# BVE-Reborn/rend3

Measured on AMD Instinct MI355X. Metric: shaded Mpixels/s @4K (whole frame: cull+compact all cameras, 4 shadow views, PBR opaque, tonemap), higher is better.
Workload: dtype f32; 1 GPU; BASELINE.json configs[2] stand-in: bistro_like (seed 0xB157, every object owns its geometry), 3840x2160, full PBR opaque + 4 directional shadow views (2048^2), camera dolly, 130 materials with base colour + normal + AO/roughness/metallic maps (RGBA8, mips, trilinear); objects=3000, triangles=2823212, cameras=5, parallelism=single GPU

## Files before the change

rend3_amd/csrc/kernels_shade.h:

```cpp
#pragma once
#include <type_traits>

#include "device_math.h"
#include "texture.h"

#define R3N_TEX_OCC 5
#define R3N_MS_OCC 4

struct TriRecord;
struct ViewLights;
struct ShadeArgs {
    const unsigned long long *vis;
    uint32_t width, height, row_begin, row_end;
    const r3n_frame_uniforms496 *fu;
    const r3n_camera_header240 *hdr;
    const r3n_object128 *objects;
    const uint32_t *mesh;
    const r3n_baked128 *baked;
    const r3n_material208 *materials;
    uint32_t n_materials;
    const uint32_t *tri_base;
    const uint32_t *slot_table;
    uint32_t slot_table_size;
    const uint8_t *dir_buf;
    const uint8_t *point_buf;
    const float *atlas;
    uint32_t atlas_w, atlas_h;
    float clear[4];
    ushort4 *hdr_out;
    uchar4 *ldr_out;
    const unsigned char *srgb_lut;
    bool out_bgr;
    TextureArgs tex;
    ushort4 *samples_out;
    TriRecord *tri_rec;
    unsigned char *seen;
    uint32_t total_tris;
    uint32_t *edge_list, *edge_count;
    uint32_t edge_capacity;
    const ViewLights *view_lights;
    const uint32_t *material_feat;
    uint32_t variants;
    uint32_t resolve_lds;
};
#define R3N_EDGEQ 32u

#define R3N_FEAT_TEX_ALBEDO   0x001u
#define R3N_FEAT_TEX_NORMAL   0x002u
#define R3N_FEAT_TEX_AOMR     0x004u
#define R3N_FEAT_TEX_AOMR_X   0x008u
#define R3N_FEAT_TEX_MISC     0x010u
#define R3N_FEAT_VCOLOR       0x020u
#define R3N_FEAT_UNLIT        0x040u
#define R3N_FEAT_NEAREST      0x080u
#define R3N_FEAT_AOMR_SPLIT   0x100u
#define R3N_FEAT_CLEARCOAT    0x200u
#define R3N_FEAT_NORMAL_FLAGS 0x400u
#define R3N_FEAT_ALBEDO_OFF   0x800u
#define R3N_FEAT_TEX_GENERAL  0x1000u
#define R3N_FEAT_ALL          0x1FFFu
#define R3N_BATCH_OCC 4
#define R3N_CLS_PLAIN  0u
#define R3N_CLS_ALBEDO (R3N_FEAT_TEX_ALBEDO)
#define R3N_CLS_PBR3   (R3N_FEAT_TEX_ALBEDO | R3N_FEAT_TEX_NORMAL | R3N_FEAT_TEX_AOMR)
#define R3N_CLS_ALL    R3N_FEAT_ALL
#define R3N_VARIANTS 4u
static inline uint32_t r3n_material_features(const r3n_material208 &m) {
    const uint32_t f = m.flags;
    uint32_t k = 0;
    if (m.textures[0]) k |= R3N_FEAT_TEX_ALBEDO;
    if (m.textures[1]) k |= R3N_FEAT_TEX_NORMAL;
    if (m.textures[2]) k |= R3N_FEAT_TEX_AOMR;
    if (m.textures[3] || m.textures[9]) k |= R3N_FEAT_TEX_AOMR_X;
    if (m.textures[4] || m.textures[5] || m.textures[6] || m.textures[7]) k |= R3N_FEAT_TEX_MISC;
    if (f & R3N_FLAGS_ALBEDO_BLEND) k |= R3N_FEAT_VCOLOR;
    if (f & R3N_FLAGS_UNLIT) k |= R3N_FEAT_UNLIT;
    if (f & R3N_FLAGS_NEAREST) k |= R3N_FEAT_NEAREST;
    if ((m.textures[2] || m.textures[3] || m.textures[9]) && !(f & R3N_FLAGS_AOMR_COMBINED)) k |= R3N_FEAT_AOMR_SPLIT;
    if (!(m.clear_coat == 0.0f)) k |= R3N_FEAT_CLEARCOAT;
    if (f & (R3N_FLAGS_BICOMPONENT_NORMAL | R3N_FLAGS_SWIZZLED_NORMAL | R3N_FLAGS_YDOWN_NORMAL)) k |= R3N_FEAT_NORMAL_FLAGS;
    if (!(f & R3N_FLAGS_ALBEDO_ACTIVE)) k |= R3N_FEAT_ALBEDO_OFF;
    return k;
}
#if defined(__HIPCC__)
__host__ __device__
#endif
static inline uint32_t r3n_variant_of(uint32_t feat) {
    if (feat & ~R3N_CLS_PBR3) return 3u;
    if (feat & ~R3N_CLS_ALBEDO) return 2u;
    return feat ? 1u : 0u;
}

struct TriRecord {
    float e[3][3];
    float vp[3][4];
    float vn[3][3];
    float vt[3][3];
    float vc[3][4];
    float uv[3][2];
    uint32_t object, material;
    uint32_t feat;
    uint32_t _pad[4];
};
static_assert(sizeof(TriRecord) == 256, "triangle record is 64 dwords");

struct BlendApplyArgs {
    const unsigned long long *keys;
    const uint32_t *vals;
    const uint32_t *head;
    uint32_t first_sample, n_samples;
    uint32_t capacity;
    ushort4 *samples;
};

#define R3N_SRGB_LUT_SIZE 0x3C00u

struct LdsDirLight {
    float m[16];
    float l[3];
    float color[3];
    float inv_res[2], offset[2], size[2];
    float sane;
    float _pad[3];
};
static_assert(sizeof(LdsDirLight) == 128, "two s_load_dwordx16");
struct LdsPointLight {
    float vpos[3];
    float color[3];
    float radius;
    float _pad;
};
static_assert(sizeof(LdsPointLight) == 32, "one s_load_dwordx8");
struct ViewLights {
    uint32_t n_dir, n_point, _pad[2];
    LdsDirLight dir[R3N_MAX_DIR_LIGHTS];
    LdsPointLight point[R3N_MAX_POINT_LIGHTS];
};

#ifndef R3N_SHADE_DECL_ONLY

struct PcfTap {
    int ix, iy;
    float fx, fy;
};
R3N_DEV PcfTap pcf_tap(uint32_t aw, uint32_t ah, float u, float v, int ox, int oy) {
    const float tx = (u * (float)aw - 0.5f) + (float)ox;
    const float ty = (v * (float)ah - 0.5f) + (float)oy;
    const float fx0 = floorf(tx), fy0 = floorf(ty);
    PcfTap t;
    t.fx = tx - fx0; t.fy = ty - fy0;
    t.ix = (fx0 == fx0 && fabsf(fx0) < 1e9f) ? (int)fx0 : 0;
    t.iy = (fy0 == fy0 && fabsf(fy0) < 1e9f) ? (int)fy0 : 0;
    if (!(t.fx == t.fx)) t.fx = 0.0f;
    if (!(t.fy == t.fy)) t.fy = 0.0f;
    return t;
}
R3N_DEV uint32_t wrap_texel(int v, uint32_t n) {
    if ((uint32_t)v < n) return (uint32_t)v;
    const long long w = (long long)n;
    return (uint32_t)((((long long)v % w) + w) % w);
}
R3N_DEV float pcf_texel_cmp(const float *__restrict__ atlas, uint32_t aw, uint32_t ah, int x, int y, float ref) {
    return ref >= atlas[(size_t)wrap_texel(y, ah) * aw + wrap_texel(x, aw)] ? 1.0f : 0.0f;
}

template <class M>
R3N_DEV float shadow_pcf5_general(const float *__restrict__ atlas, uint32_t aw, uint32_t ah, float u, float v, float ref) {
    float r = 0.0f;
#pragma unroll 1
    for (int k = 0; k < 5; ++k) {
        const int ox = k == 3 ? 1 : (k == 4 ? -1 : 0), oy = k == 1 ? 1 : (k == 2 ? -1 : 0);
        const PcfTap t = pcf_tap(aw, ah, u, v, ox, oy);
        float c[4];
#pragma unroll 1
        for (int j = 0; j < 4; ++j) c[j] = pcf_texel_cmp(atlas, aw, ah, t.ix + (j & 1), t.iy + (j >> 1), ref);
        const f2 tb = M::mad((f2){c[1], c[3]}, splat2(t.fx), (f2){c[0], c[2]} * splat2(1.0f - t.fx));
        r = r + M::mad(tb.y, t.fy, tb.x * (1.0f - t.fy));
    }
    return r * 0.2f;
}

template <class M>
R3N_DEV float shadow_pcf5(const float *__restrict__ atlas, uint32_t aw, uint32_t ah, float u, float v, float ref) {
    const float tx0 = u * (float)aw - 0.5f, ty0 = v * (float)ah - 0.5f;
    const float txp = tx0 + 1.0f, txm = tx0 + -1.0f, typ = ty0 + 1.0f, tym = ty0 + -1.0f;
    const float f0x = floorf(tx0), fpx = floorf(txp), fmx = floorf(txm);
    const float f0y = floorf(ty0), fpy = floorf(typ), fmy = floorf(tym);
// ... 69 lines not shown
    const float x = 1.0f - loh, x2 = x * x, x5 = (x2 * x2) * x;
    const float ggxl = nov * M::sqrt(M::mad(M::mad(-nol, a2, nol), nol, a2));
    const float ggxv = nol * (pre ? pre->sqrt_v : M::sqrt(M::mad(M::mad(-nov, a2, nov), nov, a2)));
    const float vis = M::half_over(ggxl + ggxv);
    const float k = nol * occlusion;
    const float dv = d * vis;
    {
        const f2 f0 = {px.f0[0], px.f0[1]};
        const f2 fres = M::mad(splat2(f90) - f0, splat2(x5), f0);
        const f2 color = M::mad(splat2(dv), fres, (f2){px.diffuse[0], px.diffuse[1]} * splat2(1.0f / R3N_PI));
        const f2 o = (color * (f2){intensity[0], intensity[1]}) * splat2(k);
        out[0] = o.x; out[1] = o.y;
    }
    {
        const float fres = M::mad(f90 - px.f0[2], x5, px.f0[2]);
        const float color = M::mad(dv, fres, px.diffuse[2] * (1.0f / R3N_PI));
        out[2] = (color * intensity[2]) * k;
    }
}

R3N_DEV float srgb_to_linear(float e) { return e > 0.04045f ? powf((e + 0.055f) / 1.055f, 2.4f) : e / 12.92f; }

R3N_DEV float srgb_oetf(float x) {
    if (!(x > 0.0f)) return 0.0f;
    if (x >= 1.0f) return 1.0f;
    if (x <= 0.0031308f) return x * 12.92f;
    return 1.055f * powf(x, 1.0f / 2.4f) - 0.055f;
}
static __global__ __launch_bounds__(256) void k_build_srgb_lut(unsigned char *__restrict__ lut) {
    const uint32_t h = blockIdx.x * 256u + threadIdx.x;
    if (h >= R3N_SRGB_LUT_SIZE) return;
    const float x = (float)__builtin_bit_cast(_Float16, (unsigned short)h);
    lut[h] = (unsigned char)(srgb_oetf(x) * 255.0f + 0.5f);
}
R3N_DEV unsigned char srgb8_of_half(const unsigned char *__restrict__ lut, unsigned short h) {
    if (h & 0x8000u) return 0;
    if (h > 0x7C00u) return 0;
    if (h >= R3N_SRGB_LUT_SIZE) return 255;
    return lut[h];
}
R3N_DEV uchar4 tonemap_half4(const unsigned char *__restrict__ lut, ushort4 h, bool bgr = false) {
    const float al = (float)__builtin_bit_cast(_Float16, h.w);
    const float a = (!(al > 0.0f)) ? 0.0f : (al >= 1.0f ? 1.0f : al);
    const unsigned char r = srgb8_of_half(lut, h.x), g = srgb8_of_half(lut, h.y), b = srgb8_of_half(lut, h.z);
    return make_uchar4(bgr ? b : r, g, bgr ? r : b, (unsigned char)(a * 255.0f + 0.5f));
}
R3N_DEV float srgb_scene_to_display(float x) {
    const float e = x > 0.0031308f ? 1.055f * powf(x, 0.4166f) - 0.055f : x * 12.92f;
    if (!(e > 0.0f)) return 0.0f;
    return e >= 1.0f ? 1.0f : e;
}

R3N_DEV ushort4 pack_half4(const float v[4]) {
    ushort4 o;
    o.x = __builtin_bit_cast(unsigned short, (_Float16)v[0]);
    o.y = __builtin_bit_cast(unsigned short, (_Float16)v[1]);
    o.z = __builtin_bit_cast(unsigned short, (_Float16)v[2]);
    o.w = __builtin_bit_cast(unsigned short, (_Float16)v[3]);
    return o;
}


template <bool TEX>
R3N_DEV void vertex_stage(const ShadeArgs &a, uint32_t id, TriRecord &r) {
    const uint32_t slot = id - 1u;
    const uint32_t bucket = slot >> R3N_SLOT_TABLE_SHIFT;
    uint32_t lo = a.slot_table[bucket];
    uint32_t hi = bucket + 1u < a.slot_table_size ? a.slot_table[bucket + 1u] + 1u : a.hdr->object_count;
    while (hi - lo > 1u) {
        const uint32_t mid = lo + (hi - lo) / 2u;
        if (a.tri_base[mid] <= slot) lo = mid; else hi = mid;
    }
    const uint32_t obj = lo, tri = slot - a.tri_base[obj];
    const r3n_object128 &ob = a.objects[obj];
    const uint4 of0 = *reinterpret_cast<const uint4 *>(reinterpret_cast<const char *>(&ob) + 80);
    const uint4 of1 = *reinterpret_cast<const uint4 *>(reinterpret_cast<const char *>(&ob) + 96);
    const uint32_t of5 = ob.vertex_attribute_start_offsets[5];
    const uint32_t mat_index = of0.z < a.n_materials ? of0.z : 0u;
    const r3n_material208 &mat = a.materials[mat_index];
    const float *mv = a.baked[obj].model_view;
    r.object = obj;
    r.material = mat_index;
    r.feat = a.material_feat != nullptr ? a.material_feat[mat_index] : R3N_FEAT_ALL;

    uint32_t idx[3];
    float p[3][4];
    const float inv_s2[3] = {1.0f / dot3(mv, mv), 1.0f / dot3(mv + 4, mv + 4), 1.0f / dot3(mv + 8, mv + 8)};
    const uint32_t first = of0.x + tri * 3u;
    const uint32_t pos_off = of0.w;
    const uint32_t nrm_off = of1.x;
    const uint32_t tan_off = of1.y;
    const uint32_t uv0_off = of1.z;
    const uint32_t col_off = of5;
    bool any_tex = false, normal_map = false;
    if (TEX) {
        const uint4 t0 = *reinterpret_cast<const uint4 *>(&mat.textures[0]), t1 = *reinterpret_cast<const uint4 *>(&mat.textures[4]);
        const uint2 t2 = *reinterpret_cast<const uint2 *>(&mat.textures[8]);
        any_tex = (((t0.x | t0.y) | (t0.z | t0.w)) | ((t1.x | t1.y) | (t1.z | t1.w)) | (t2.x | t2.y)) != 0u;
        normal_map = t0.y != 0u;
    }
    fetch_indices3(a.mesh, first, idx);
#pragma unroll
    for (int k = 0; k < 3; ++k) {
        float v[3];
        fetch_vec3(a.mesh, pos_off, idx[k], v);
        mul_point(a.baked[obj].model_view_proj, v, p[k]);
        mul_point(mv, v, r.vp[k]);
        float nm[3] = {0.0f, 0.0f, 0.0f};
        if (nrm_off != R3N_INVALID) fetch_vec3(a.mesh, nrm_off, idx[k], nm);
        const float sn[3] = {inv_s2[0] * nm[0], inv_s2[1] * nm[1], inv_s2[2] * nm[2]};
        mat3_mul_vec3(mv, mv + 4, mv + 8, sn, r.vn[k]);
        normalize3(r.vn[k]);
        if (TEX && normal_map) {
            float tg[3] = {0.0f, 0.0f, 0.0f};
            if (tan_off != R3N_INVALID) fetch_vec3(a.mesh, tan_off, idx[k], tg);
            const float st[3] = {inv_s2[0] * tg[0], inv_s2[1] * tg[1], inv_s2[2] * tg[2]};
            mat3_mul_vec3(mv, mv + 4, mv + 8, st, r.vt[k]);
            normalize3(r.vt[k]);
        } else {
            r.vt[k][0] = r.vt[k][1] = r.vt[k][2] = 0.0f;
        }
        if (col_off != R3N_INVALID) {
            const uint32_t cw = a.mesh[col_off / 4u + idx[k]];
#pragma unroll
            for (int c = 0; c < 4; ++c) r.vc[k][c] = (float)((cw >> (8 * c)) & 0xFFu) / 255.0f;
        } else {
#pragma unroll
            for (int c = 0; c < 4; ++c) r.vc[k][c] = 1.0f;
        }
        if (TEX && any_tex) fetch_uv0(a.mesh, uv0_off, idx[k], r.uv[k]);
        else r.uv[k][0] = r.uv[k][1] = 0.0f;
    }
    TriSetup ts;
    setup_triangle(p, (float)a.width / 2.0f, (float)a.height / 2.0f,
                   (a.hdr->flags & R3N_PCU_POSITIVE_AREA_VISIBLE) != 0u, ts);
#pragma unroll
    for (int i = 0; i < 3; ++i)
#pragma unroll
        for (int c = 0; c < 3; ++c) r.e[i][c] = ts.e[i][c];
}

template <class M> R3N_DEV f2 interp2(const float lam[3], f2 a0, f2 a1, f2 a2) {
    return M::mad(splat2(lam[2]), a2, M::mad(splat2(lam[1]), a1, splat2(lam[0]) * a0));
}
template <class M> R3N_DEV float interp1(const float lam[3], float a0, float a1, float a2) {
    return M::mad(lam[2], a2, M::mad(lam[1], a1, lam[0] * a0));
}
template <class M> R3N_DEV void interp_vec3(const float lam[3], const float a[3][3], float o[3]) {
    const f2 xy = interp2<M>(lam, (f2){a[0][0], a[0][1]}, (f2){a[1][0], a[1][1]}, (f2){a[2][0], a[2][1]});
    o[0] = xy.x; o[1] = xy.y;
    o[2] = interp1<M>(lam, a[0][2], a[1][2], a[2][2]);
}
template <class M> R3N_DEV void interp_vec4(const float lam[3], const float a[3][4], float o[4]) {
    const f2 xy = interp2<M>(lam, (f2){a[0][0], a[0][1]}, (f2){a[1][0], a[1][1]}, (f2){a[2][0], a[2][1]});
    const f2 zw = interp2<M>(lam, (f2){a[0][2], a[0][3]}, (f2){a[1][2], a[1][3]}, (f2){a[2][2], a[2][3]});
    o[0] = xy.x; o[1] = xy.y; o[2] = zw.x; o[3] = zw.y;
}

template <class T, bool SL> R3N_DEV T load_light(const T *p) {
#if defined(__HIP_DEVICE_COMPILE__)
    if (SL) {
        static_assert(sizeof(T) % 4 == 0, "whole dwords");
        const unsigned long long v = (unsigned long long)p;
        const uint32_t lo = (uint32_t)__builtin_amdgcn_readfirstlane((uint32_t)v), hi = (uint32_t)__builtin_amdgcn_readfirstlane((uint32_t)(v >> 32));
        typedef __attribute__((address_space(4))) const uint32_t *sp_t;
        const sp_t sp = (sp_t)(((unsigned long long)hi << 32) | (unsigned long long)lo);
        union { T t; uint32_t w[sizeof(T) / 4]; } u;
#pragma unroll
        for (unsigned k = 0; k < sizeof(T) / 4; ++k) u.w[k] = sp[k];
        return u.t;
    }
#endif
    return *p;
}
template <bool TEX, class M = MathExact, uint32_t CLS = R3N_CLS_ALL, bool SL = false>
R3N_DEV void fragment_stage(const ShadeArgs &a, const LdsDirLight *s_dir, const LdsPointLight *s_point, uint32_t n_dir,
                            uint32_t n_point, const TriRecord &r, uint32_t x, uint32_t y, float out[4]) {
    const r3n_material208 &mat = a.materials[r.material];
    constexpr bool kVColor = (CLS & R3N_FEAT_VCOLOR) != 0u, kUnlit = (CLS & R3N_FEAT_UNLIT) != 0u, kNearest = (CLS & R3N_FEAT_NEAREST) != 0u;
    constexpr bool kSplit = (CLS & R3N_FEAT_AOMR_SPLIT) != 0u, kNormalFlags = (CLS & R3N_FEAT_NORMAL_FLAGS) != 0u;
    constexpr bool kAlbedoOff = (CLS & R3N_FEAT_ALBEDO_OFF) != 0u, kMisc = (CLS & R3N_FEAT_TEX_MISC) != 0u;
    constexpr bool kClearCoat = (CLS & (R3N_FEAT_CLEARCOAT | R3N_FEAT_TEX_MISC)) != 0u;
    constexpr bool kAnyTex = TEX && (CLS & (R3N_FEAT_TEX_ALBEDO | R3N_FEAT_TEX_NORMAL | R3N_FEAT_TEX_AOMR | R3N_FEAT_TEX_AOMR_X | R3N_FEAT_TEX_MISC)) != 0u;
    constexpr uint32_t kSlotFeat[10] = {R3N_FEAT_TEX_ALBEDO, R3N_FEAT_TEX_NORMAL, R3N_FEAT_TEX_AOMR, R3N_FEAT_TEX_AOMR_X, R3N_FEAT_TEX_MISC,
                                        R3N_FEAT_TEX_MISC, R3N_FEAT_TEX_MISC, R3N_FEAT_TEX_MISC, R3N_FEAT_TEX_MISC ,
                                        R3N_FEAT_TEX_AOMR_X};
    TriSetup ts;
#pragma unroll
    for (int i = 0; i < 3; ++i)
#pragma unroll
        for (int c = 0; c < 3; ++c) ts.e[i][c] = r.e[i][c];
    ts.z[0] = ts.z[1] = ts.z[2] = 0.0f; ts.det = 1.0f; ts.valid = true;
    float E[3];
    (void)edge_eval(ts, (float)x + 0.5f, (float)y + 0.5f, E);
    const float rs = exact_math::rcp((E[0] + E[1]) + E[2]);
    const float lam[3] = {E[0] * rs, E[1] * rs, E[2] * rs};
    float vpos[4], nrm[3], col[4] = {1.0f, 1.0f, 1.0f, 1.0f};
    interp_vec4<MathExact>(lam, r.vp, vpos);
    interp_vec3<M>(lam, r.vn, nrm);
    if (kVColor && (mat.flags & R3N_FLAGS_ALBEDO_ACTIVE) && (mat.flags & R3N_FLAGS_ALBEDO_BLEND))
        interp_vec4<M>(lam, r.vc, col);

    PixelData px;
    const uint32_t mflags = mat.flags;
    bool any_tex = false;
    if (kAnyTex) {
#pragma unroll
        for (int k = 0; k < 10; ++k)
            if (CLS & kSlotFeat[k]) any_tex = any_tex || mat.textures[k] != 0u;
    }
    float coords[2] = {0.0f, 0.0f}, ddx[2] = {0.0f, 0.0f}, ddy[2] = {0.0f, 0.0f};
    const bool nearest = kNearest && (mflags & R3N_FLAGS_NEAREST) != 0u;
    if (kAnyTex && any_tex) {
        const f2 sr = interp2<M>(lam, (f2){r.uv[0][0], r.uv[0][1]}, (f2){r.uv[1][0], r.uv[1][1]}, (f2){r.uv[2][0], r.uv[2][1]});
        const float self_raw[2] = {sr.x, sr.y};
        frag_coords<M>(ts, r.uv, mat.uv_transform0, (int)x, (int)y, coords, ddx, ddy, self_raw);
    }
    constexpr bool kShortOnly = (CLS & (R3N_FEAT_TEX_GENERAL | R3N_FEAT_NEAREST)) == 0u;
    constexpr bool kShare = kShortOnly && (CLS & (R3N_FEAT_TEX_NORMAL | R3N_FEAT_TEX_AOMR)) != 0u;
    TexShare tshare;
    tshare.width = 0u; tshare.height = 0u; tshare.mips = 0u; tshare.level = 0u; tshare.frac = 0.0f;
    auto tex4 = [&](int slot, float dst[4]) { tex_sample_grad<M, true, kShortOnly, kShare>(a.tex, mat.textures[slot], nearest, coords[0], coords[1], ddx, ddy, dst, &tshare); };
    auto tex3 = [&](int slot, float dst[4]) { tex_sample_grad<M, false, kShortOnly, kShare>(a.tex, mat.textures[slot], nearest, coords[0], coords[1], ddx, ddy, dst, &tshare); };
    auto has = [&](int slot) { return TEX && (CLS & kSlotFeat[slot]) != 0u && mat.textures[slot] != 0u; };
    constexpr bool kBatch = TEX && kShortOnly && CLS == R3N_CLS_PBR3;
    float tb3[3][4];
    bool batched = false;
    if (kBatch && any_tex) {
        const uint32_t ids[3] = {mat.textures[0], mat.textures[1], mat.textures[2]};
        batched = tex_sample3_batched<M>(a.tex, ids, coords[0], coords[1], ddx, ddy, tb3);
    }
    auto tex_slot012 = [&](int slot, float dst[4], bool need_a) {
        if (kBatch && batched) {
#pragma unroll
            for (int c = 0; c < 4; ++c) dst[c] = tb3[slot][c];
        } else if (need_a) tex4(slot, dst);
        else tex3(slot, dst);
    };
    if (!kAlbedoOff || (mflags & R3N_FLAGS_ALBEDO_ACTIVE)) {
#pragma unroll
        for (int c = 0; c < 4; ++c) px.albedo[c] = 1.0f;
        if (has(0)) tex_slot012(0, px.albedo, true);
        if (kVColor && (mflags & R3N_FLAGS_ALBEDO_BLEND)) {
            if (mflags & R3N_FLAGS_ALBEDO_VERTEX_SRGB) {
#pragma unroll
                for (int c = 0; c < 3; ++c) px.albedo[c] *= srgb_to_linear(col[c]);
                px.albedo[3] *= col[3];
            } else {
#pragma unroll
                for (int c = 0; c < 4; ++c) px.albedo[c] *= col[c];
            }
        }
    } else {
        px.albedo[0] = px.albedo[1] = px.albedo[2] = 0.0f;
        px.albedo[3] = 1.0f;
    }
    {
        const f2 rg = (f2){px.albedo[0], px.albedo[1]} * (f2){mat.albedo[0], mat.albedo[1]};
        const f2 ba = (f2){px.albedo[2], px.albedo[3]} * (f2){mat.albedo[2], mat.albedo[3]};
        px.albedo[0] = rg.x; px.albedo[1] = rg.y; px.albedo[2] = ba.x; px.albedo[3] = ba.y;
    }

    if (kUnlit && (mflags & R3N_FLAGS_UNLIT)) {
#pragma unroll
        for (int c = 0; c < 4; ++c) out[c] = px.albedo[c];
    } else {
        if (has(1)) {
            float t[4], n[3];
            tex_slot012(1, t, true);
            if (kNormalFlags && (mflags & R3N_FLAGS_BICOMPONENT_NORMAL)) {
                float b0 = (mflags & R3N_FLAGS_SWIZZLED_NORMAL) ? t[3] : t[0], b1 = t[1];
                b0 = M::mad(b0, 2.0f, -1.0f);
                b1 = M::mad(b1, 2.0f, -1.0f);
                n[0] = b0; n[1] = b1;
                n[2] = M::sqrt((1.0f - b0 * b0) - b1 * b1);
            } else {
#pragma unroll
                for (int c = 0; c < 3; ++c) n[c] = M::mad(t[c], 2.0f, -1.0f);
                normalize3m<M>(n);
            }
            if (kNormalFlags && (mflags & R3N_FLAGS_YDOWN_NORMAL)) n[1] = -n[1];
            float tng[3];
            interp_vec3<M>(lam, r.vt, tng);
            float nn[3] = {nrm[0], nrm[1], nrm[2]};
            normalize3m<M>(nn);
            normalize3m<M>(tng);
            const float bt[3] = {nn[1] * tng[2] - tng[1] * nn[2], nn[2] * tng[0] - tng[2] * nn[0], nn[0] * tng[1] - tng[0] * nn[1]};
            mat3_mul_vec3m<M>(tng, bt, nn, n, px.normal);
        } else {
#pragma unroll
            for (int c = 0; c < 3; ++c) px.normal[c] = nrm[c];
        }
        normalize3m<M>(px.normal);
        float ao = mat.ambient_occlusion, pr = mat.roughness, metallic = mat.metallic;
        if (!kSplit || (mflags & R3N_FLAGS_AOMR_COMBINED)) {
            if (has(2)) {
                float t[4];
                tex_slot012(2, t, false);
                ao = mat.ambient_occlusion * t[0];
                pr = mat.roughness * t[1];
                metallic = mat.metallic * t[2];
            }
        } else if (mflags & R3N_FLAGS_AOMR_BW_SPLIT) {
            float t[4];
            if (has(2)) { tex3(2, t); pr = mat.roughness * t[0]; }
            if (has(3)) { tex3(3, t); metallic = mat.metallic * t[0]; }
            if (has(9)) { tex3(9, t); ao = mat.ambient_occlusion * t[0]; }
        } else {
            float t[4];
            if (has(2)) {
                tex3(2, t);
                const bool sw = (mflags & R3N_FLAGS_AOMR_SWIZZLED_SPLIT) != 0u;
                pr = mat.roughness * (sw ? t[1] : t[0]);
                metallic = mat.metallic * (sw ? t[2] : t[1]);
// ... 46 lines not shown
#pragma unroll
        for (int c = 0; c < 3; ++c) vv[c] = -vv[c];
        float color[3] = {px.emissive[0], px.emissive[1], px.emissive[2]};
        const float mag = (((fabsf(px.normal[0]) + fabsf(px.normal[1])) + (fabsf(px.normal[2]) + fabsf(vv[0]))) +
                           ((fabsf(vv[1]) + fabsf(vv[2])) + (fabsf(px.f0[0]) + fabsf(px.f0[1])))) +
                          (((fabsf(px.f0[2]) + fabsf(px.diffuse[0])) + (fabsf(px.diffuse[1]) + fabsf(px.diffuse[2]))) + fabsf(px.ao));
        const bool skip_ok = px.roughness >= 1e-9f && px.roughness <= 1e9f && mag < 1e30f;
        const BrdfPixel pre_v = brdf_pixel<M>(px, vv);
        const BrdfPixel *pre = &pre_v;
        for (uint32_t i = 0; i < n_dir; ++i) {
            const LdsDirLight L = load_light<LdsDirLight, SL>(s_dir + i);
            const float nl_raw = dot3m<M>(px.normal, L.l);
            if (px.roughness > 0.0f && nl_raw == nl_raw && sat(nl_raw) == 0.0f) {
#pragma unroll
                for (int c = 0; c < 3; ++c) color[c] += 0.0f;
                continue;
            }
            float sn[4];
            mul_vec4m<MathExact>(L.m, vpos[0], vpos[1], vpos[2], vpos[3], sn);
            const float fl[2] = {sn[0] * 0.5f + 0.5f, sn[1] * 0.5f + 0.5f};
            const float local[2] = {fl[0], 1.0f - fl[1]};
            float tl[2] = {L.offset[0], L.offset[1]};
            float tr[2] = {tl[0] + L.size[0], tl[1] + L.size[1]};
            const float coords[2] = {tl[0] * (1.0f - local[0]) + tr[0] * local[0],
                                     tl[1] * (1.0f - local[1]) + tr[1] * local[1]};
            const float border[2] = {L.inv_res[0] * 1.5f, L.inv_res[1] * 1.5f};
            tl[0] += border[0]; tl[1] += border[1];
            tr[0] -= border[0]; tr[1] -= border[1];
            float shadow = 1.0f;
            if ((fl[0] >= tl[0] || fl[1] >= tl[1]) && (fl[0] <= tr[0] || fl[1] <= tr[1]) && sn[2] >= 0.0f && sn[2] <= 1.0f)
                shadow = shadow_pcf5<M>(a.atlas, a.atlas_w, a.atlas_h, coords[0], coords[1], sn[2]);
            if (skip_ok && L.sane != 0.0f && shadow * px.ao == 0.0f) {
#pragma unroll
                for (int c = 0; c < 3; ++c) color[c] += 0.0f;
                continue;
            }
            float res[3];
            surface_shading<M>(L.l, L.color, px, vv, shadow * px.ao, res, pre);
#pragma unroll
            for (int c = 0; c < 3; ++c) color[c] += res[c];
        }
        for (uint32_t i = 0; i < n_point; ++i) {
            const LdsPointLight P = load_light<LdsPointLight, SL>(s_point + i);
            const float delta[3] = {P.vpos[0] - vpos[0], P.vpos[1] - vpos[1], P.vpos[2] - vpos[2]};
            const float d = M::sqrt(dot3m<M>(delta, delta));
            const float s = sat(M::div(d, P.radius));
            const float s2 = s * s, is2 = 1.0f - s2;
            const float att = M::div(is2 * is2, 1.0f + s2);
            const float inten[3] = {P.color[0] * att, P.color[1] * att, P.color[2] * att};
            const float l[3] = {M::div(delta[0], d), M::div(delta[1], d), M::div(delta[2], d)};
            float res[3];
            surface_shading<M>(l, inten, px, vv, px.ao, res, pre);
#pragma unroll
            for (int c = 0; c < 3; ++c) color[c] += (res[c] > 0.0f ? res[c] : 0.0f);
        }
#pragma unroll
        for (int c = 0; c < 3; ++c) out[c] = fmaxf(a.fu->ambient[c] * px.albedo[c], color[c]);
        out[3] = fmaxf(a.fu->ambient[3] * px.albedo[3], px.albedo[3]);
    }
}

template <bool TEX, class M = MathExact>
R3N_DEV void shade_fragment(const ShadeArgs &a, const LdsDirLight *s_dir, const LdsPointLight *s_point, uint32_t n_dir,
                            uint32_t n_point, uint32_t id, uint32_t x, uint32_t y, float out[4]) {
    TriRecord r;
    vertex_stage<TEX>(a, id, r);
    fragment_stage<TEX, M>(a, s_dir, s_point, n_dir, n_point, r, x, y, out);
}

static __global__ __launch_bounds__(256) void k_mark_visible(const unsigned long long *__restrict__ vis, unsigned char *__restrict__ seen,
                                                      size_t first_pixel, size_t n_pixels) {
    const size_t i = (size_t)blockIdx.x * 256u + threadIdx.x;
    const uint32_t id = i < n_pixels ? (uint32_t)(vis[first_pixel + i] & 0xFFFFFFFFull) : 0u;
    const uint32_t left = (uint32_t)__builtin_amdgcn_update_dpp((int)~id, (int)id, 0x111, 0xF, 0xF, false);
    if (id != 0u && id != left) seen[id - 1u] = 1;
}
template <bool TEX>
__global__ __launch_bounds__(256) void k_vertex_stage(ShadeArgs a) {
    const uint32_t slot = blockIdx.x * 256u + threadIdx.x;
    if (slot >= a.total_tris || !a.seen[slot]) return;
    a.seen[slot] = 0;
    TriRecord r;
    vertex_stage<TEX>(a, slot + 1u, r);
    r._pad[0] = r._pad[1] = r._pad[2] = r._pad[3] = 0u;
    a.tri_rec[slot] = r;
}

R3N_DEV void stage_lights(const ShadeArgs &a, LdsDirLight *s_dir, LdsPointLight *s_point, uint32_t &n_dir, uint32_t &n_point) {
    n_dir = min(*reinterpret_cast<const uint32_t *>(a.dir_buf), (uint32_t)R3N_MAX_DIR_LIGHTS);
    n_point = min(*reinterpret_cast<const uint32_t *>(a.point_buf), (uint32_t)R3N_MAX_POINT_LIGHTS);

    const r3n_dir_light128 *dirs = reinterpret_cast<const r3n_dir_light128 *>(a.dir_buf + 16);
    const r3n_point_light32 *points = reinterpret_cast<const r3n_point_light32 *>(a.point_buf + 16);
    for (uint32_t i = threadIdx.x; i < n_dir * 4u; i += 256u) {
        const uint32_t li = i >> 2, c = i & 3u;
        const float *col = a.fu->inv_view + 4 * c;
        float o[4];
        mul_vec4(dirs[li].view_proj, col[0], col[1], col[2], col[3], o);
#pragma unroll
        for (int r = 0; r < 4; ++r) s_dir[li].m[4 * c + r] = o[r];
        if (c == 0) {
            const float nd[3] = {-dirs[li].direction[0], -dirs[li].direction[1], -dirs[li].direction[2]};
            float l[3];
            mat3_mul_vec3(a.fu->view, a.fu->view + 4, a.fu->view + 8, nd, l);
            normalize3(l);
#pragma unroll
            for (int r = 0; r < 3; ++r) { s_dir[li].l[r] = l[r]; s_dir[li].color[r] = dirs[li].color[r]; }
            s_dir[li].sane = (fabsf(dirs[li].color[0]) <= 1e6f && fabsf(dirs[li].color[1]) <= 1e6f && fabsf(dirs[li].color[2]) <= 1e6f &&
                              fabsf(l[0]) <= 2.0f && fabsf(l[1]) <= 2.0f && fabsf(l[2]) <= 2.0f) ? 1.0f : 0.0f;
#pragma unroll
            for (int r = 0; r < 2; ++r) {
                s_dir[li].inv_res[r] = dirs[li].inv_resolution[r];
                s_dir[li].offset[r] = dirs[li].atlas_offset[r];
                s_dir[li].size[r] = dirs[li].atlas_size[r];
            }
        }
    }
    for (uint32_t i = threadIdx.x; i < n_point; i += 256u) {
        float o[4];
        mul_vec4(a.fu->view, points[i].position[0], points[i].position[1], points[i].position[2], points[i].position[3], o);
#pragma unroll
        for (int r = 0; r < 3; ++r) { s_point[i].vpos[r] = o[r]; s_point[i].color[r] = points[i].color[r]; }
        s_point[i].radius = points[i].radius;
    }
    __syncthreads();
}

static __global__ __launch_bounds__(256) void k_stage_view_lights(ShadeArgs a, ViewLights *out) {
    uint32_t n_dir, n_point;
    stage_lights(a, out->dir, out->point, n_dir, n_point);
    if (threadIdx.x == 0u) { out->n_dir = n_dir; out->n_point = n_point; out->_pad[0] = out->_pad[1] = 0u; }
}

template <int S, bool TEX, bool REC = false, bool SPLIT = false, bool FAST = false, uint32_t CLS = R3N_CLS_ALL, uint32_t VARIANT = 3u>
__global__ __launch_bounds__(256, (S == 1 && !TEX) ? 5 : (REC ? (S == 1 ? (CLS == R3N_CLS_PBR3 ? R3N_BATCH_OCC : R3N_TEX_OCC) : R3N_MS_OCC) : 1)) void k_resolve_opaque(ShadeArgs a) {
    typedef typename std::conditional<FAST, MathFast, MathExact>::type M;
    static_assert(CLS == R3N_CLS_ALL || (S == 1 && REC), "material classes exist for the single-sample record-based resolve");
    __shared__ LdsDirLight s_dir[R3N_MAX_DIR_LIGHTS];
    __shared__ LdsPointLight s_point[R3N_MAX_POINT_LIGHTS];
    __shared__ float s_decode[512];
    const uint32_t wv = threadIdx.x >> 6, ln = threadIdx.x & 63u;
    const uint32_t bx = blockIdx.x, by = blockIdx.y;
    const uint32_t x = bx * 16u + (ln & 7u) + 8u * (wv & 1u);
    const uint32_t y = a.row_begin + by * 16u + (ln >> 3) + 8u * (wv >> 1);
    const bool inside = x < a.width && y < a.row_end;
    const size_t pix = inside ? (size_t)y * a.width + x : 0u;
    uint32_t id1 = 0u;
    if (S == 1) {
        id1 = inside ? (uint32_t)(a.vis[pix] & 0xFFFFFFFFull) : 0u;
        if (REC && (a.variants & (a.variants - 1u)) != 0u) {
            __shared__ uint32_t s_feat;
            if (threadIdx.x == 0u) s_feat = 0u;
            __syncthreads();
            uint32_t f = id1 ? a.tri_rec[id1 - 1u].feat : 0u;
#pragma unroll
            for (int d = 1; d < 64; d <<= 1) f |= __shfl_xor(f, d);
            if (ln == 0u && f) atomicOr(&s_feat, f);
            __syncthreads();
            uint32_t v = r3n_variant_of(s_feat);
            while (v < R3N_VARIANTS - 1u && !((a.variants >> v) & 1u)) ++v;
            if (v != VARIANT) return;
        }
    }
    if (TEX) {
        s_decode[threadIdx.x] = a.tex.decode[threadIdx.x];
        s_decode[256u + threadIdx.x] = a.tex.decode[256u + threadIdx.x];
        a.tex.decode = s_decode;
// ... 321 lines not shown
```

rend3_amd/csrc/texture.h:

```cpp
#pragma once
#include "device_math.h"


struct TextureArgs {
    const r3n_texture_desc32 *descs;
    uint32_t count;
    const uint32_t *texels;
    const float *decode;
    const uint32_t *level_off;
    uint32_t small_pool;
};

R3N_DEV uint32_t tex_mip_dim(uint32_t d, uint32_t k) {
    const uint32_t v = d >> k;
    return v ? v : 1u;
}
R3N_DEV uint32_t tex_wrap(float f, uint32_t n) {
    const int i = (f == f && fabsf(f) < 1e9f) ? (int)f : 0;
    if ((uint32_t)i < n) return (uint32_t)i;
    if ((n & (n - 1u)) == 0u) return (uint32_t)i & (n - 1u);
    const int m = i % (int)n;
    return (uint32_t)(m < 0 ? m + (int)n : m);
}
R3N_DEV uint32_t tex_level_start_pow2(uint32_t W, uint32_t H, uint32_t L) {
// ... 245 lines not shown
        }
        if (level >= d.mips - 1u) { level = d.mips - 1u; frac = 0.0f; }
        const float *rgb = t.decode + (d.format == 1u ? 256 : 0);
        const uint32_t w0 = tex_mip_dim(d.width, level), h0 = tex_mip_dim(d.height, level);
        const uint32_t *lo = t.level_off + (size_t)(id - 1u) * R3N_TEX_LEVELS;
        const uint32_t b0 = SHORT_ONLY ? d.offset + tex_level_start_pow2(d.width, d.height, level) : lo[level];
        TexLvlFast l0, l1;
        bool tame = tex_level_fast<SHORT_ONLY>(w0, h0, b0, u, v, l0);
        const bool two = frac > 0.0f;
        if (two) tame = tex_level_fast<SHORT_ONLY>(tex_mip_dim(d.width, level + 1u), tex_mip_dim(d.height, level + 1u), SHORT_ONLY ? b0 + __umul24(w0, h0) : lo[level + 1u], u, v, l1) && tame;
        if (SHORT_ONLY || tame) {
            Texel4 r, hi;
            r = tex_bilinear_fast<M, NEED_A>(t, rgb, l0);
            if (two) hi = tex_bilinear_fast<M, NEED_A>(t, rgb, l1);
            if (two) {
                const float omf = 1.0f - frac;
                r.rg = mix2<M>(r.rg, hi.rg, frac, omf);
                if (NEED_A) r.ba = mix2<M>(r.ba, hi.ba, frac, omf);
                else r.ba.x = M::mad(hi.ba.x, frac, r.ba.x * omf);
            }
            o[0] = r.rg.x; o[1] = r.rg.y; o[2] = r.ba.x; o[3] = r.ba.y;
            return;
        }
    }
    if (SHORT_ONLY) return;
    TexFootprint f;
    tex_footprint(d, nearest, u, v, ddx, ddy, f);
    const Texel4 r = tex_apply<M, NEED_A>(t, d, f);
    o[0] = r.rg.x; o[1] = r.rg.y; o[2] = r.ba.x; o[3] = r.ba.y;
}

template <class M = MathExact, bool SHORT_ONLY = false>
R3N_DEV float tex_sample_alpha(const TextureArgs &t, uint32_t id, const r3n_texture_desc32 &d, bool nearest, float u, float v, const float ddx[2], const float ddy[2]) {
    if (id == 0u || id > t.count) return 0.0f;
    const bool pow2 = (((d.width & (d.width - 1u)) | (d.height & (d.height - 1u))) == 0u);
    if (SHORT_ONLY || (!nearest && pow2 && t.small_pool != 0u && d.format < R3N_POOL_FLOAT)) {
        const float W = (float)d.width, H = (float)d.height;
        const float ax = ddx[0] * W, ay = ddx[1] * H, bx = ddy[0] * W, by = ddy[1] * H;
        const float rho = exact_math::sqrt(fmaxf(ax * ax + ay * ay, bx * bx + by * by));
        uint32_t level = 0;
        float frac = 0.0f;
        if (rho > 1.0f && rho < INFINITY) {
            const uint32_t bits = __float_as_uint(rho);
            level = (bits >> 23) - 127u;
            frac = (float)(bits & 0x7FFFFFu) / 8388608.0f;
        } else if (rho == INFINITY) {
            level = d.mips;
        }
        if (level >= d.mips - 1u) { level = d.mips - 1u; frac = 0.0f; }
        const uint32_t w0 = tex_mip_dim(d.width, level), h0 = tex_mip_dim(d.height, level);
        const uint32_t *lo = t.level_off + (size_t)(id - 1u) * R3N_TEX_LEVELS;
        const uint32_t b0 = SHORT_ONLY ? d.offset + tex_level_start_pow2(d.width, d.height, level) : lo[level];
        TexLvlFast l0, l1;
        bool tame = tex_level_fast<SHORT_ONLY>(w0, h0, b0, u, v, l0);
        const bool two = frac > 0.0f;
        if (two) tame = tex_level_fast<SHORT_ONLY>(tex_mip_dim(d.width, level + 1u), tex_mip_dim(d.height, level + 1u), SHORT_ONLY ? b0 + __umul24(w0, h0) : lo[level + 1u], u, v, l1) && tame;
        if (SHORT_ONLY || tame) {
            const char *pool = reinterpret_cast<const char *>(t.texels);
            auto byte_at = [&](uint32_t byte_off) { return *reinterpret_cast<const uint32_t *>(pool + byte_off) >> 24; };
            const uint32_t c00 = byte_at(l0.o00), c10 = byte_at(l0.o10), c01 = byte_at(l0.o01), c11 = byte_at(l0.o11);
            uint32_t d00 = c00, d10 = c10, d01 = c01, d11 = c11;
            if (two) { d00 = byte_at(l1.o00); d10 = byte_at(l1.o10); d01 = byte_at(l1.o01); d11 = byte_at(l1.o11); }
            const uint32_t all_and = (c00 & c10) & (c01 & c11) & (d00 & d10) & (d01 & d11);
            const uint32_t all_or = (c00 | c10) | (c01 | c11) | (d00 | d10) | (d01 | d11);
            if (all_and == 255u) return 1.0f;
            if (all_or == 0u) return 0.0f;
            auto bilinear = [&](const TexLvlFast &l, uint32_t b00, uint32_t b10, uint32_t b01, uint32_t b11) {
                const float a00 = exact_math::unorm8(b00), a10 = exact_math::unorm8(b10), a01 = exact_math::unorm8(b01), a11 = exact_math::unorm8(b11);
                const float omx = 1.0f - l.fx, omy = 1.0f - l.fy;
                const float top = M::mad(a10, l.fx, a00 * omx), bot = M::mad(a11, l.fx, a01 * omx);
                return M::mad(bot, l.fy, top * omy);
            };
            float r = bilinear(l0, c00, c10, c01, c11);
            if (two) r = M::mad(bilinear(l1, d00, d10, d01, d11), frac, r * (1.0f - frac));
            return r;
        }
    }
    if (SHORT_ONLY) return 0.0f;
    float o[4];
    tex_sample_grad<M, true>(t, id, nearest, u, v, ddx, ddy, o);
    return o[3];
}

template <class M>
R3N_DEV bool tex_sample3_batched(const TextureArgs &t, const uint32_t id[3], float u, float v, const float ddx[2], const float ddy[2],
                                 float out[3][4]) {
    bool present[3];
    uint32_t w[3], h[3], mips[3], fmt[3], base[3];
#pragma unroll
    for (int k = 0; k < 3; ++k) {
        present[k] = id[k] != 0u;
        const uint32_t idx = present[k] ? id[k] - 1u : 0u;
        const uint4 dw = *reinterpret_cast<const uint4 *>(&t.descs[idx]);
        base[k] = dw.x; w[k] = dw.y; h[k] = dw.z; mips[k] = dw.w;
        fmt[k] = t.descs[idx].format;
    }
    uint32_t W = 0u, H = 0u, MI = 0u;
#pragma unroll
    for (int k = 0; k < 3; ++k)
        if (present[k] && w[k] > W) { W = w[k]; H = h[k]; MI = mips[k]; }
    bool ok = true, any_half = false, half[3];
#pragma unroll
    for (int k = 0; k < 3; ++k) {
        const bool same = w[k] == W && h[k] == H && mips[k] == MI;
        half[k] = present[k] && !same && (w[k] << 1) == W && (h[k] << 1) == H && mips[k] + 1u == MI;
        ok = ok && (!present[k] || same || half[k]);
        any_half = any_half || half[k];
    }
    if (!__all(ok)) return false;
    uint32_t level = 0;
    float frac = 0.0f;
    {
        const float Wf = (float)W, Hf = (float)H;
        const float ax = ddx[0] * Wf, ay = ddx[1] * Hf, bx = ddy[0] * Wf, by = ddy[1] * Hf;
        const float rho = exact_math::sqrt(fmaxf(ax * ax + ay * ay, bx * bx + by * by));
        if (rho > 1.0f && rho < INFINITY) {
            const uint32_t bits = __float_as_uint(rho);
            level = (bits >> 23) - 127u;
            frac = (float)(bits & 0x7FFFFFu) / 8388608.0f;
        } else if (rho == INFINITY) {
            level = MI;
        }
        if (MI != 0u && level >= MI - 1u) { level = MI - 1u; frac = 0.0f; }
    }
    TexLvlRel f0, f1;
    tex_level_rel(tex_mip_dim(W, level), tex_mip_dim(H, level), u, v, f0);
    const bool need1 = frac > 0.0f || (any_half && level == 0u);
    f1 = f0;
    if (need1) tex_level_rel(tex_mip_dim(W, level + 1u), tex_mip_dim(H, level + 1u), u, v, f1);
    uint32_t la[3], ba[3], bb[3];
    bool first_is_f1[3], two[3];
#pragma unroll
    for (int k = 0; k < 3; ++k) {
        first_is_f1[k] = half[k] && level == 0u;
        la[k] = half[k] ? (level == 0u ? 0u : level - 1u) : level;
        two[k] = frac > 0.0f && !first_is_f1[k];
    }
#pragma unroll
    for (int k = 0; k < 3; ++k) {
        ba[k] = base[k] + tex_level_start_pow2(w[k], h[k], la[k]);
        bb[k] = two[k] ? ba[k] + __umul24(tex_mip_dim(w[k], la[k]), tex_mip_dim(h[k], la[k])) : ba[k];
        if (!present[k]) { ba[k] = 0u; bb[k] = 0u; }
    }
    struct __attribute__((packed, aligned(4))) W2 { uint32_t v[2]; };
    uint32_t ta[3][4], tb[3][4];
    const char *pool = reinterpret_cast<const char *>(t.texels);
    const bool any_two = __any(frac > 0.0f);
    const bool pair0 = f0.r10 == f0.r00 + 1u, pair1 = f1.r10 == f1.r00 + 1u;
    bool wrap_a = false;
#pragma unroll
    for (int k = 0; k < 3; ++k) {
        const TexLvlRel &fa = first_is_f1[k] ? f1 : f0;
        const W2 top = *reinterpret_cast<const W2 *>(pool + ((ba[k] + fa.r00) << 2));
        const W2 bot = *reinterpret_cast<const W2 *>(pool + ((ba[k] + fa.r01) << 2));
        ta[k][0] = top.v[0]; ta[k][1] = top.v[1]; ta[k][2] = bot.v[0]; ta[k][3] = bot.v[1];
        wrap_a = wrap_a || !(first_is_f1[k] ? pair1 : pair0);
    }
    if (__any(wrap_a)) {
#pragma unroll
        for (int k = 0; k < 3; ++k) {
            const TexLvlRel &fa = first_is_f1[k] ? f1 : f0;
            if (!(first_is_f1[k] ? pair1 : pair0)) {
                ta[k][1] = *reinterpret_cast<const uint32_t *>(pool + ((ba[k] + fa.r10) << 2));
                ta[k][3] = *reinterpret_cast<const uint32_t *>(pool + ((ba[k] + fa.r11) << 2));
            }
        }
    }
    uint32_t ob[3][4];
    bool pair_b[3], wrap_b = false;
#pragma unroll
    for (int k = 0; k < 3; ++k) {
        const bool use1 = two[k] || first_is_f1[k];
        const TexLvlRel &fb = use1 ? f1 : f0;
        ob[k][0] = (bb[k] + fb.r00) << 2; ob[k][1] = (bb[k] + fb.r10) << 2; ob[k][2] = (bb[k] + fb.r01) << 2; ob[k][3] = (bb[k] + fb.r11) << 2;
        pair_b[k] = use1 ? pair1 : pair0;
        wrap_b = wrap_b || !pair_b[k];
    }
    asm volatile("" : : "v"(ob[0][0]), "v"(ob[1][0]), "v"(ob[2][0]));
// ... 94 lines not shown
```

Before: 9648 Mpixels/s.

## Precompute per-triangle texture descriptors and UV transform into triangle record

For triangles whose material falls in the PBR3 class, the vertex stage now packs the three texture descriptors (offset, size, mips, format, presence bit) and the UV transform into the triangle record. It reuses the vertex-colour slot and padding through a union. The fragment stage reads this per-triangle state instead of gathering material texture ids and descriptors for every pixel. This removes dependent global loads per pixel in exchange for more vertex-stage work, and it assumes widths, heights and mip counts fit in 16 bits.

Result: no change. 9804 Mpixels/s, median of 6 (+1.6%).

```diff
diff --git a/rend3_amd/csrc/kernels_shade.h b/rend3_amd/csrc/kernels_shade.h
--- a/rend3_amd/csrc/kernels_shade.h
+++ b/rend3_amd/csrc/kernels_shade.h
@@ -91,18 +91,26 @@
     return feat ? 1u : 0u;
 }
 
+struct TriTexState {
+    float uvt[6];
+    TexDesc3 desc;
+    uint32_t _pad;
+};
 struct TriRecord {
     float e[3][3];
     float vp[3][4];
     float vn[3][3];
     float vt[3][3];
-    float vc[3][4];
     float uv[3][2];
     uint32_t object, material;
     uint32_t feat;
-    uint32_t _pad[4];
+    union {
+        float vc[3][4];
+        TriTexState tex;
+    };
 };
 static_assert(sizeof(TriRecord) == 256, "triangle record is 64 dwords");
+static_assert(sizeof(TriTexState) == 64 && offsetof(TriRecord, tex) == 192, "sampling state: the record's last 16 dwords");
 
 struct BlendApplyArgs {
     const unsigned long long *keys;
@@ -338,6 +346,8 @@
     r.object = obj;
     r.material = mat_index;
     r.feat = a.material_feat != nullptr ? a.material_feat[mat_index] : R3N_FEAT_ALL;
+    const bool tex_state = TEX && (r.feat & ~R3N_CLS_PBR3) == 0u;
+    r.tex = TriTexState{};
 
     uint32_t idx[3];
     float p[3][4];
@@ -349,8 +359,10 @@
     const uint32_t uv0_off = of1.z;
     const uint32_t col_off = of5;
     bool any_tex = false, normal_map = false;
+    uint4 t0 = {0u, 0u, 0u, 0u};
     if (TEX) {
-        const uint4 t0 = *reinterpret_cast<const uint4 *>(&mat.textures[0]), t1 = *reinterpret_cast<const uint4 *>(&mat.textures[4]);
+        t0 = *reinterpret_cast<const uint4 *>(&mat.textures[0]);
+        const uint4 t1 = *reinterpret_cast<const uint4 *>(&mat.textures[4]);
         const uint2 t2 = *reinterpret_cast<const uint2 *>(&mat.textures[8]);
         any_tex = (((t0.x | t0.y) | (t0.z | t0.w)) | ((t1.x | t1.y) | (t1.z | t1.w)) | (t2.x | t2.y)) != 0u;
         normal_map = t0.y != 0u;
@@ -376,16 +388,24 @@
         } else {
             r.vt[k][0] = r.vt[k][1] = r.vt[k][2] = 0.0f;
         }
-        if (col_off != R3N_INVALID) {
-            const uint32_t cw = a.mesh[col_off / 4u + idx[k]];
-#pragma unroll
-            for (int c = 0; c < 4; ++c) r.vc[k][c] = (float)((cw >> (8 * c)) & 0xFFu) / 255.0f;
-        } else {
-#pragma unroll
-            for (int c = 0; c < 4; ++c) r.vc[k][c] = 1.0f;
+        if (!tex_state) {
+            if (col_off != R3N_INVALID) {
+                const uint32_t cw = a.mesh[col_off / 4u + idx[k]];
+#pragma unroll
+                for (int c = 0; c < 4; ++c) r.vc[k][c] = (float)((cw >> (8 * c)) & 0xFFu) / 255.0f;
+            } else {
+#pragma unroll
+                for (int c = 0; c < 4; ++c) r.vc[k][c] = 1.0f;
+            }
         }
         if (TEX && any_tex) fetch_uv0(a.mesh, uv0_off, idx[k], r.uv[k]);
         else r.uv[k][0] = r.uv[k][1] = 0.0f;
+    }
+    if (tex_state) {
+        const float *m = mat.uv_transform0;
+        r.tex.uvt[0] = m[0]; r.tex.uvt[1] = m[1]; r.tex.uvt[2] = m[4]; r.tex.uvt[3] = m[5]; r.tex.uvt[4] = m[8]; r.tex.uvt[5] = m[9];
+        const uint32_t ids[3] = {t0.x, t0.y, t0.z};
+        tex_desc3_pack(a.tex, ids, r.tex.desc);
     }
     TriSetup ts;
     setup_triangle(p, (float)a.width / 2.0f, (float)a.height / 2.0f,
@@ -441,6 +461,15 @@
     constexpr uint32_t kSlotFeat[10] = {R3N_FEAT_TEX_ALBEDO, R3N_FEAT_TEX_NORMAL, R3N_FEAT_TEX_AOMR, R3N_FEAT_TEX_AOMR_X, R3N_FEAT_TEX_MISC,
                                         R3N_FEAT_TEX_MISC, R3N_FEAT_TEX_MISC, R3N_FEAT_TEX_MISC, R3N_FEAT_TEX_MISC ,
                                         R3N_FEAT_TEX_AOMR_X};
+    constexpr bool kBatch = TEX && CLS == R3N_CLS_PBR3;
+    TriTexState tx = {};
+    float uv_pre[3][2] = {};
+    if (kBatch) {
+        tx = r.tex;
+#pragma unroll
+        for (int i = 0; i < 3; ++i) { uv_pre[i][0] = r.uv[i][0]; uv_pre[i][1] = r.uv[i][1]; }
+    }
+    const float (*const uv)[2] = kBatch ? uv_pre : r.uv;
     TriSetup ts;
 #pragma unroll
     for (int i = 0; i < 3; ++i)
@@ -459,8 +488,11 @@
 
     PixelData px;
     const uint32_t mflags = mat.flags;
+    auto bound = [&](int slot) { return slot < 3 && (tx.desc.mf[slot] >> 31) != 0u; };
     bool any_tex = false;
-    if (kAnyTex) {
+    if (kBatch) {
+        any_tex = ((tx.desc.mf[0] | tx.desc.mf[1] | tx.desc.mf[2]) >> 31) != 0u;
+    } else if (kAnyTex) {
 #pragma unroll
         for (int k = 0; k < 10; ++k)
             if (CLS & kSlotFeat[k]) any_tex = any_tex || mat.textures[k] != 0u;
@@ -468,9 +500,11 @@
     float coords[2] = {0.0f, 0.0f}, ddx[2] = {0.0f, 0.0f}, ddy[2] = {0.0f, 0.0f};
     const bool nearest = kNearest && (mflags & R3N_FLAGS_NEAREST) != 0u;
     if (kAnyTex && any_tex) {
-        const f2 sr = interp2<M>(lam, (f2){r.uv[0][0], r.uv[0][1]}, (f2){r.uv[1][0], r.uv[1][1]}, (f2){r.uv[2][0], r.uv[2][1]});
+        const f2 sr = interp2<M>(lam, (f2){uv[0][0], uv[0][1]}, (f2){uv[1][0], uv[1][1]}, (f2){uv[2][0], uv[2][1]});
         const float self_raw[2] = {sr.x, sr.y};
-        frag_coords<M>(ts, r.uv, mat.uv_transform0, (int)x, (int)y, coords, ddx, ddy, self_raw);
+        const float *t = tx.uvt;
+        const float uvt[10] = {t[0], t[1], 0.0f, 0.0f, t[2], t[3], 0.0f, 0.0f, t[4], t[5]};
+        frag_coords<M>(ts, uv, kBatch ? uvt : mat.uv_transform0, (int)x, (int)y, coords, ddx, ddy, self_raw);
     }
     constexpr bool kShortOnly = (CLS & (R3N_FEAT_TEX_GENERAL | R3N_FEAT_NEAREST)) == 0u;
     constexpr bool kShare = kShortOnly && (CLS & (R3N_FEAT_TEX_NORMAL | R3N_FEAT_TEX_AOMR)) != 0u;
@@ -478,14 +512,10 @@
     tshare.width = 0u; tshare.height = 0u; tshare.mips = 0u; tshare.level = 0u; tshare.frac = 0.0f;
     auto tex4 = [&](int slot, float dst[4]) { tex_sample_grad<M, true, kShortOnly, kShare>(a.tex, mat.textures[slot], nearest, coords[0], coords[1], ddx, ddy, dst, &tshare); };
     auto tex3 = [&](int slot, float dst[4]) { tex_sample_grad<M, false, kShortOnly, kShare>(a.tex, mat.textures[slot], nearest, coords[0], coords[1], ddx, ddy, dst, &tshare); };
-    auto has = [&](int slot) { return TEX && (CLS & kSlotFeat[slot]) != 0u && mat.textures[slot] != 0u; };
-    constexpr bool kBatch = TEX && kShortOnly && CLS == R3N_CLS_PBR3;
+    auto has = [&](int slot) { return TEX && (CLS & kSlotFeat[slot]) != 0u && (kBatch ? bound(slot) : mat.textures[slot] != 0u); };
     float tb3[3][4];
     bool batched = false;
-    if (kBatch && any_tex) {
-        const uint32_t ids[3] = {mat.textures[0], mat.textures[1], mat.textures[2]};
-        batched = tex_sample3_batched<M>(a.tex, ids, coords[0], coords[1], ddx, ddy, tb3);
-    }
+    if (kBatch && any_tex) batched = tex_sample3_batched<M>(a.tex, tx.desc, coords[0], coords[1], ddx, ddy, tb3);
     auto tex_slot012 = [&](int slot, float dst[4], bool need_a) {
         if (kBatch && batched) {
 #pragma unroll
@@ -698,7 +728,6 @@
     a.seen[slot] = 0;
     TriRecord r;
     vertex_stage<TEX>(a, slot + 1u, r);
-    r._pad[0] = r._pad[1] = r._pad[2] = r._pad[3] = 0u;
     a.tri_rec[slot] = r;
 }
 
diff --git a/rend3_amd/csrc/texture.h b/rend3_amd/csrc/texture.h
--- a/rend3_amd/csrc/texture.h
+++ b/rend3_amd/csrc/texture.h
@@ -351,18 +351,33 @@
     return o[3];
 }
 
+struct TexDesc3 {
+    uint32_t offset[3];
+    uint32_t wh[3];
+    uint32_t mf[3];
+};
+R3N_DEV void tex_desc3_pack(const TextureArgs &t, const uint32_t id[3], TexDesc3 &o) {
+#pragma unroll
+    for (int k = 0; k < 3; ++k) {
+        const bool present = id[k] != 0u;
+        const uint32_t idx = present ? id[k] - 1u : 0u;
+        const uint4 dw = *reinterpret_cast<const uint4 *>(&t.descs[idx]);
+        o.offset[k] = dw.x;
+        o.wh[k] = dw.y | dw.z << 16;
+        o.mf[k] = dw.w | t.descs[idx].format << 16 | (present ? 0x80000000u : 0u);
+    }
+}
+
 template <class M>
-R3N_DEV bool tex_sample3_batched(const TextureArgs &t, const uint32_t id[3], float u, float v, const float ddx[2], const float ddy[2],
+R3N_DEV bool tex_sample3_batched(const TextureArgs &t, const TexDesc3 &d, float u, float v, const float ddx[2], const float ddy[2],
                                  float out[3][4]) {
     bool present[3];
     uint32_t w[3], h[3], mips[3], fmt[3], base[3];
 #pragma unroll
     for (int k = 0; k < 3; ++k) {
-        present[k] = id[k] != 0u;
-        const uint32_t idx = present[k] ? id[k] - 1u : 0u;
-        const uint4 dw = *reinterpret_cast<const uint4 *>(&t.descs[idx]);
-        base[k] = dw.x; w[k] = dw.y; h[k] = dw.z; mips[k] = dw.w;
-        fmt[k] = t.descs[idx].format;
+        present[k] = (d.mf[k] >> 31) != 0u;
+        base[k] = d.offset[k]; w[k] = d.wh[k] & 0xFFFFu; h[k] = d.wh[k] >> 16;
+        mips[k] = d.mf[k] & 0xFFFFu; fmt[k] = (d.mf[k] >> 16) & 0x7FFFu;
     }
     uint32_t W = 0u, H = 0u, MI = 0u;
 #pragma unroll
```
